# coecms/xmhw

Measured on AMD Instinct MI355X. Metric: grid-cells/sec for threshold() on 40yr daily SST, higher is better.
Workload: dtype f32 in / f64 out; 1 GPU; 0.25deg global (configs[2]): 1036800 cells per step, 1982-2021 (T=14610), windowHalfWidth=5, pctile=90, smoothPercentileWidth=31, nan_frac=0.0, skipna=False; cells_rank0=1036800, T=14610, D=366, kernel=clim_sorted_f32 (sorted row-lists in LDS, 2 lanes per cell, layout 40), slabs=1, gather=none

## Files before the change

### include/xmhw_amd.h

```cpp
#ifndef XMHW_AMD_H
#define XMHW_AMD_H

#include <stddef.h>
#include <stdint.h>

#ifdef __cplusplus
extern "C" {
#endif

#define XMHW_OK 0
#define XMHW_ERR_INVALID 1
#define XMHW_ERR_HIP 2
#define XMHW_ERR_UNSUPPORTED 3
#define XMHW_ERR_NOMEM 4
#define XMHW_ERR_COMM 5

#define XMHW_KERNEL_AUTO 0
#define XMHW_KERNEL_RING 1
#define XMHW_KERNEL_GENERIC 2

int xmhw_version(void);
const char *xmhw_arch(void);
const char *xmhw_last_error(void);
int xmhw_device_count(int *count);
// ... 72 lines not shown
    XMHW_LAYOUT_RING2_4LANE = 10,
    XMHW_LAYOUT_RING2_16LANE = 12,
    XMHW_LAYOUT_RING3_8LANE = 20,
    XMHW_LAYOUT_RING3_4LANE = 21,
    XMHW_LAYOUT_RING3_2LANE = 22,
    XMHW_LAYOUT_SORTED = 40
};
int xmhw_plan_set_layout(xmhw_plan *plan, int32_t layout);
int xmhw_plan_layout_in_use(const xmhw_plan *plan, int32_t *layout);
int xmhw_sorted_device_ok(int32_t *holds);
int xmhw_plan_set_ring2(xmhw_plan *plan, int32_t variant);
int xmhw_plan_ring2_in_use(const xmhw_plan *plan, int32_t *variant);
int xmhw_plan_f64_mode(const xmhw_plan *plan, int32_t *variant);
enum { XMHW_ROUTE_GENERIC = 0, XMHW_ROUTE_RING1 = 1, XMHW_ROUTE_RING2 = 2, XMHW_ROUTE_RING3 = 3, XMHW_ROUTE_RING4 = 4,
       XMHW_ROUTE_SORTED = 5 };
#define XMHW_ROUTE_WORDS 25
int xmhw_plan_route(const xmhw_plan *plan, int32_t elem_bytes, double q, int64_t C, int32_t *out, int32_t n);

int xmhw_clim_raw_f32(xmhw_plan *plan, const float *ts_dev, int64_t C, int64_t ld,
                      double q, int negate, double *thresh_dev, double *seas_dev,
                      int64_t ldo, void *stream);
int xmhw_clim_raw_f64(xmhw_plan *plan, const double *ts_dev, int64_t C, int64_t ld,
                      double q, int negate, double *thresh_dev, double *seas_dev,
                      int64_t ldo, void *stream);
int xmhw_clim_raw_i16(xmhw_plan *plan, const int16_t *codes_dev, int64_t C, int64_t ld, int big_endian,
                      int has_scale, double scale_factor, double add_offset, int has_fill, int32_t fill_code,
                      int decoded_itemsize, double q, int negate, double *thresh_dev, double *seas_dev,
                      int64_t ldo, void *stream);

int xmhw_clim_finish(const xmhw_plan *plan, const double *thresh_in_dev,
                     const double *seas_in_dev, int64_t C, int64_t ldo, int feb29_fix,
                     int smooth, int smooth_width, double *thresh_out_dev,
                     double *seas_out_dev, void *stream);

int xmhw_clim_f32(const float *ts_dev, const int32_t *doy_host, int64_t T, int64_t C,
                  int32_t D, int32_t window_half_width, double q, int smooth,
                  int smooth_width, int feb29_fix, int negate, double *thresh_dev,
                  double *seas_dev, void *stream);
int xmhw_clim_f64(const double *ts_dev, const int32_t *doy_host, int64_t T, int64_t C,
                  int32_t D, int32_t window_half_width, double q, int smooth,
                  int smooth_width, int feb29_fix, int negate, double *thresh_dev,
                  double *seas_dev, void *stream);
int xmhw_clim_host_f32(const float *ts_host, const int32_t *doy_host, int64_t T, int64_t C,
                       int32_t D, int32_t window_half_width, double q, int smooth,
                       int smooth_width, int feb29_fix, int negate, double *thresh_host,
                       double *seas_host);
int xmhw_clim_host_f64(const double *ts_host, const int32_t *doy_host, int64_t T, int64_t C,
                       int32_t D, int32_t window_half_width, double q, int smooth,
                       int smooth_width, int feb29_fix, int negate, double *thresh_host,
                       double *seas_host);

int xmhw_land_mask_f32(const float *ts_dev, int64_t T, int64_t C, int64_t ld, int anynans,
                       uint8_t *keep_dev, void *stream);
int xmhw_land_mask_f64(const double *ts_dev, int64_t T, int64_t C, int64_t ld, int anynans,
                       uint8_t *keep_dev, void *stream);

int xmhw_land_mask_i16(const int16_t *codes_dev, int64_t T, int64_t C, int64_t ld, int big_endian, int has_fill,
                       int32_t fill_code, int anynans, uint8_t *keep_dev, void *stream);

int xmhw_gather_cells_f32(const float *in_dev, int64_t rows, int64_t ld_in,
                          const int64_t *index_dev, int64_t n, float *out_dev, int64_t ld_out,
                          void *stream);
int xmhw_gather_cells_f64(const double *in_dev, int64_t rows, int64_t ld_in,
                          const int64_t *index_dev, int64_t n, double *out_dev, int64_t ld_out,
                          void *stream);
int xmhw_gather_cells_i16(const int16_t *in_dev, int64_t rows, int64_t ld_in,
// ... 436 lines not shown
```

### xmhw_amd/csrc/capi.cpp

```cpp
#include "../../include/xmhw_amd.h"

#include <hip/hip_runtime.h>
#include <unistd.h>

#include <cerrno>
#include <cmath>

#include <algorithm>
#include <cstdio>
#include <cstdlib>
#include <atomic>
#include <cstring>
#include <map>
#include <memory>
#include <mutex>
#include <new>
#include <string>
#include <vector>

#include "kernels.h"
#include "plan.h"
#include "route.h"
#include "stage_blocks.h"

// ... 1702 lines not shown
        pk.s = scale_factor;
        pk.o = add_offset;
        pk.val_neg = negate ? 1 : 0;
        kneg = (negate ? 1 : 0) ^ (scale_factor < 0.0 ? 1 : 0);
    }
    pk.key_neg = kneg;
    Ready rd;
    const int rc = ensure(plan, route, C, true, &rd);
    if (rc != XMHW_OK) return rc;
    hipStream_t st = static_cast<hipStream_t>(stream);
    const xmhw::Plan& h = plan->host;
    const hipError_t e = timed_launch(rd, st, [&] {
        return xmhw::launch_sorted_i16(codes, pk, C, ld, h.T, rd.table[0], rd.dev.sflags_s, rd.dev.chunks_s, rd.dev.nchunks_s, h.w,
                                       route.launch[0].tpl, h.ntracks, q, kneg, thresh, seas, ldo, st);
    });
    if (e != hipSuccess) return hip_fail(e, "packed climatology launch");
    return XMHW_OK;
}

int xmhw_clim_finish(const xmhw_plan* plan, const double* thresh_in, const double* seas_in, int64_t C,
                     int64_t ldo, int feb29_fix, int smooth, int smooth_width, double* thresh_out,
                     double* seas_out, void* stream) {
    if (!plan) return fail(XMHW_ERR_INVALID, "plan is NULL");
    if (smooth && (smooth_width <= 0 || smooth_width % 2 == 0))
        return fail(XMHW_ERR_INVALID, "Running average window should be odd");
    if (C < 0 || ldo < C) return fail(XMHW_ERR_INVALID, "bad C/ldo");
    if (C == 0) return XMHW_OK;
    if (!thresh_in || !seas_in || !thresh_out || !seas_out)
        return fail(XMHW_ERR_INVALID, "NULL device buffer");
    if (thresh_in == thresh_out || seas_in == seas_out)
        return fail(XMHW_ERR_INVALID, "in and out may not alias");
    const xmhw::Plan& h = plan->host;
    ScratchRef flags;
    if (smooth && smooth_width == 31)
        if (int rc = claim_scratch(static_cast<hipStream_t>(stream), static_cast<size_t>(C), &flags)) return rc;
    return status_of(xmhw::launch_finish(thresh_in, seas_in, C, ldo, h.D, row_index(h, 59), row_index(h, 60),
                                         row_index(h, 61), feb29_fix, smooth, smooth ? smooth_width : 1, thresh_out,
                                         seas_out, static_cast<hipStream_t>(stream), static_cast<uint8_t*>(flags.get())),
                     "clim_finish launch");
}

int xmhw_clim_f32(const float* ts, const int32_t* doy, int64_t T, int64_t C, int32_t D, int32_t w,
                  double q, int smooth, int smooth_w, int feb29_fix, int negate, double* thresh,
                  double* seas, void* stream) {
    return clim_oneshot<float>(ts, doy, T, C, D, w, q, smooth, smooth_w, feb29_fix, negate, thresh, seas,
                               stream);
}
int xmhw_clim_f64(const double* ts, const int32_t* doy, int64_t T, int64_t C, int32_t D, int32_t w,
                  double q, int smooth, int smooth_w, int feb29_fix, int negate, double* thresh,
                  double* seas, void* stream) {
    return clim_oneshot<double>(ts, doy, T, C, D, w, q, smooth, smooth_w, feb29_fix, negate, thresh, seas,
                                stream);
}
int xmhw_clim_host_f32(const float* ts, const int32_t* doy, int64_t T, int64_t C, int32_t D, int32_t w,
                       double q, int smooth, int smooth_w, int feb29_fix, int negate, double* thresh,
                       double* seas) {
    return clim_host<float>(ts, doy, T, C, D, w, q, smooth, smooth_w, feb29_fix, negate, thresh, seas);
}
int xmhw_clim_host_f64(const double* ts, const int32_t* doy, int64_t T, int64_t C, int32_t D, int32_t w,
                       double q, int smooth, int smooth_w, int feb29_fix, int negate, double* thresh,
                       double* seas) {
    return clim_host<double>(ts, doy, T, C, D, w, q, smooth, smooth_w, feb29_fix, negate, thresh, seas);
}

int xmhw_land_mask_f32(const float* ts, int64_t T, int64_t C, int64_t ld, int anynans, uint8_t* keep,
                       void* stream) {
    if (C < 0 || ld < C || T <= 0) return fail(XMHW_ERR_INVALID, "bad T/C/ld");
    return status_of(xmhw::launch_land_mask<float>(ts, T, C, ld, anynans, keep, static_cast<hipStream_t>(stream)),
                     "land_mask launch");
}
int xmhw_land_mask_f64(const double* ts, int64_t T, int64_t C, int64_t ld, int anynans, uint8_t* keep,
                       void* stream) {
// ... 847 lines not shown
```

### xmhw_amd/csrc/kernels.h

```cpp
#pragma once
#include <hip/hip_runtime.h>
#include <stdint.h>

namespace xmhw {

struct DevChunk { int32_t warm_start, begin, end; };
struct PackedI16 {
    int32_t mode = 0;
    int32_t fill = 0x7FFFFFFF;
    int32_t swap = 0;
    int32_t key_neg = 0;
    int32_t val_neg = 0;
    float sf = 1.0f, of = 0.0f;
    double s = 1.0, o = 0.0;
};
struct DevSortedChunk { int32_t warm_start, begin, end, trow0; uint32_t direct_lo, direct_hi; };

template <typename T>
hipError_t launch_generic(const T* ts, int64_t Tn, int64_t C, int64_t ld, const int32_t* row_ptr,
                          const int32_t* centres, int32_t D, int32_t w, double q, int negate,
                          double* thresh, double* seas, int64_t ldo, hipStream_t stream,
                          const uint32_t* run_flag = nullptr);

bool ring_supported(int32_t w, int32_t yps, int32_t subs, int elem_bytes);
// ... 48 lines not shown
                             int64_t ldo, hipStream_t stream);

int32_t ring4_pick_yps(int32_t w, int32_t ntracks, int32_t subs);
bool ring4_supported(int32_t w, int32_t yps, int32_t subs);
bool ring4_stats_built();
hipError_t launch_ring4_f32(const float* ts, int64_t C, int64_t ld, int64_t Tn, const uint32_t* table,
                            const uint32_t* sflags, int32_t step_min, const DevChunk* chunks, int32_t nchunks,
                            int32_t w, int32_t yps, int32_t subs, int32_t ntracks, double q, int negate,
                            double* thresh, double* seas, int64_t ldo, hipStream_t stream,
                            unsigned long long* stats = nullptr);

bool ring3_x64_supported(int32_t w, int32_t yps, int32_t subs);
hipError_t launch_ring3_f64(const double* ts, int64_t C, int64_t ld, int64_t Tn, const uint32_t* table,
                            const uint32_t* sflags, int32_t step_min, const DevChunk* chunks, int32_t nchunks,
                            int32_t w, int32_t yps, int32_t subs, int32_t ntracks, double q, int negate, double* thresh,
                            double* seas, int64_t ldo, hipStream_t stream, const uint32_t* run_flag);
bool ring3_narrowing_supported(int32_t w, int32_t yps, int32_t subs);
hipError_t launch_ring3_f32_narrowing(const double* ts, int64_t C, int64_t ld, int64_t Tn, const uint32_t* table,
                                      const uint32_t* sflags, int32_t step_min, const DevChunk* chunks,
                                      int32_t nchunks, int32_t w, int32_t yps, int32_t subs, int32_t ntracks, double q,
                                      int negate, double* thresh, double* seas, int64_t ldo, hipStream_t stream,
                                      uint32_t* narrow_flag);

hipError_t launch_ring_f32_narrowing(const double* ts, int64_t Tn, int64_t C, int64_t ld, const uint32_t* table,
                                     int32_t step_min, const DevChunk* chunks, int32_t nchunks, int32_t w,
                                     int32_t yps, int32_t subs, double q, int negate, double* thresh, double* seas,
                                     int64_t ldo, hipStream_t stream, unsigned long long* stats,
                                     uint32_t* narrow_flag);

hipError_t launch_finish(const double* th_in, const double* se_in, int64_t C, int64_t ldo, int32_t D,
                         int32_t i59, int32_t i60, int32_t i61, int feb29_fix, int smooth,
                         int32_t width, double* th_out, double* se_out, hipStream_t stream,
                         uint8_t* flags = nullptr);

template <typename T>
hipError_t launch_land_mask(const T* ts, int64_t Tn, int64_t C, int64_t ld, int anynans,
                            uint8_t* keep, hipStream_t stream);

hipError_t launch_land_mask_i16(const int16_t* codes, int64_t Tn, int64_t C, int64_t ld, int16_t fill_raw, int anynans,
                                uint8_t* keep, hipStream_t stream);

template <typename T>
hipError_t launch_gather_cells(const T* in, int64_t rows, int64_t ld_in, const int64_t* index, int64_t n,
                               T* out, int64_t ld_out, hipStream_t stream);
hipError_t launch_scatter_cells(const double* in, int64_t rows, int64_t ld_in, const int64_t* index,
                                int64_t n, double* out, int64_t ld_out, int64_t ncols_out,
                                hipStream_t stream);

template <typename T>
hipError_t launch_detect(const T* ts, int64_t Tn, int64_t C, int64_t ld, const double* thresh, int64_t ldt,
                         const int32_t* row_of_t, int32_t min_duration, int32_t join_gaps, int32_t max_gap,
                         int32_t negate, int32_t* events, int32_t* start, int32_t* end, uint8_t* bthresh,
                         int64_t ldo, int32_t* nevents, hipStream_t stream);

hipError_t launch_count_events(const int32_t* start, int64_t Tn, int64_t C, int64_t ldo, int32_t* nevents,
                               hipStream_t stream);

constexpr int kEventColumns = 31;
template <typename T>
hipError_t launch_event_stats(const T* ts, int64_t Tn, int64_t C, int64_t ld, const double* seas,
                              const double* thresh, int64_t ldc, const int32_t* row_of_t, int32_t negate,
                              const int32_t* events, int64_t ldo, const int64_t* offsets, double* table,
                              hipStream_t stream);

hipError_t launch_floor_to_f32(const double* th, int64_t rows, int64_t cols, int64_t ldi, float* out, int64_t ldo,
                               hipStream_t stream);
// ... 313 lines not shown
```

### xmhw_amd/csrc/kernels_generic.hip

```cpp
#include "device_common.h"
#include "kernels.h"
#include "packed_src.h"

namespace xmhw {

template <typename Src>
__device__ __forceinline__ void generic_cell_row(const Src& src, int64_t c, int64_t Tn, int64_t ld,
                                                 const int32_t* __restrict__ row_ptr,
                                                 const int32_t* __restrict__ centres, int32_t row, int32_t w, double q,
                                                 int negate, double& th_out, double& se_out) {
    using T = typename Src::sample;
    using K = typename KeyOf<T>::type;
    const int32_t cb = row_ptr[row], ce = row_ptr[row + 1];

    uint32_t n = 0;
    double sum = 0.0;
    for (int32_t i = cb; i < ce; ++i) {
        const int64_t t0 = centres[i];
        for (int32_t k = -w; k <= w; ++k) {
            const int64_t t = t0 + k;
            if (t < 0 || t >= Tn) continue;
            T v = src.at(c + t * ld);
            if (negate) v = -v;
            if (v == v) { ++n; sum += static_cast<double>(v); }
        }
    }
    double th = make_nan(), se = make_nan();
    if (n > 0) {
        const double vi = static_cast<double>(n - 1) * q;
        const double fl = floor(vi);
        const uint32_t lo = static_cast<uint32_t>(fl);
        const double g = vi - fl;
// ... 52 lines not shown
    generic_cell_row(PlainSrc<T>{ts}, c, Tn, ld, row_ptr, centres, row, w, q, negate, th, se);
    thresh[static_cast<int64_t>(row) * ldo + c] = th;
    seas[static_cast<int64_t>(row) * ldo + c] = se;
}

template <typename T>
hipError_t launch_generic(const T* ts, int64_t Tn, int64_t C, int64_t ld, const int32_t* row_ptr,
                          const int32_t* centres, int32_t D, int32_t w, double q, int negate,
                          double* thresh, double* seas, int64_t ldo, hipStream_t stream,
                          const uint32_t* run_flag) {
    if (C <= 0 || D <= 0) return hipSuccess;
    dim3 grid(static_cast<unsigned>((C + 255) / 256), static_cast<unsigned>(D));
    hipLaunchKernelGGL(clim_generic<T>, grid, dim3(256), 0, stream, ts, Tn, C, ld, row_ptr, centres, w,
                       q, negate, thresh, seas, ldo, run_flag);
    return hipGetLastError();
}
template hipError_t launch_generic<float>(const float*, int64_t, int64_t, int64_t, const int32_t*,
                                          const int32_t*, int32_t, int32_t, double, int, double*,
                                          double*, int64_t, hipStream_t, const uint32_t*);
template hipError_t launch_generic<double>(const double*, int64_t, int64_t, int64_t, const int32_t*,
                                           const int32_t*, int32_t, int32_t, double, int, double*,
                                           double*, int64_t, hipStream_t, const uint32_t*);

struct FinishCol {
    const double* in;
    int64_t ld;
    int32_t i60;
    double f60;
    bool sub60;
    __device__ __forceinline__ double raw(int32_t d) const { return in[static_cast<int64_t>(d) * ld]; }
    __device__ __forceinline__ double val(int32_t d) const { return (sub60 && d == i60) ? f60 : raw(d); }
};

__global__ __launch_bounds__(256) void clim_finish(const double* __restrict__ th_in,
                                                   const double* __restrict__ se_in, int64_t C,
                                                   int64_t ld, int32_t D, int32_t i59, int32_t i60,
                                                   int32_t i61, int feb29_fix, int smooth, int32_t width,
                                                   double* __restrict__ th_out,
                                                   double* __restrict__ se_out,
                                                   const uint8_t* __restrict__ only) {
    const int64_t c = static_cast<int64_t>(blockIdx.x) * blockDim.x + threadIdx.x;
    if (c >= C) return;
    if (only != nullptr && only[c] == 0) return;
    const double* in = (blockIdx.y == 0 ? th_in : se_in) + c;
    double* out = (blockIdx.y == 0 ? th_out : se_out) + c;

    int32_t nnan = 0;
    for (int32_t d = 0; d < D; ++d) {
        const double v = in[static_cast<int64_t>(d) * ld];
        nnan += (v != v) ? 1 : 0;
    }
    FinishCol col{in, ld, i60, 0.0, false};
    if (feb29_fix && i60 >= 0) {
        const double v60 = col.raw(i60);
        if (v60 == v60) {
            double s = v60;
            int32_t m = 1;
            if (i59 >= 0) { const double v = col.raw(i59); if (v == v) { s += v; ++m; } }
            if (i61 >= 0) { const double v = col.raw(i61); if (v == v) { s += v; ++m; } }
            if (m == 3) s = (col.raw(i59) + v60) + col.raw(i61);
            else if (m == 2 && i59 >= 0 && col.raw(i59) == col.raw(i59)) s = col.raw(i59) + v60;
            col.f60 = s / static_cast<double>(m);
            col.sub60 = true;
        }
    }
    const int32_t h = (width - 1) / 2;
    const double inv = static_cast<double>(width);
    if (!smooth) {
        for (int32_t d = 0; d < D; ++d) out[static_cast<int64_t>(d) * ld] = col.val(d);
        return;
    }
    if (nnan == 0) {
        int32_t trail = ((-h) % D + D) % D;
        int32_t lead = trail;
        double s = -0.0;
        for (int32_t i = 0; i < width; ++i) {
            s += col.val(lead);
            if (i + 1 < width) lead = (lead + 1 == D) ? 0 : lead + 1;
        }
// ... 40 lines not shown
    for (int32_t i = 0; i < width; ++i) {
        s += col.val(lead);
        if (i + 1 < width) lead = next_present(lead);
    }
    double fresh = -0.0;
    int32_t nfresh = 0;
    int32_t cur = first;
    for (int32_t d = 0; d < first; ++d) out[static_cast<int64_t>(d) * ld] = make_nan();
    for (int32_t j = 0; j < np; ++j) {
        out[static_cast<int64_t>(cur) * ld] = s / inv;
        s -= col.val(trail);
        trail = next_present(trail);
        lead = next_present(lead);
        const double v = col.val(lead);
        s += v;
        fresh += v;
        if (++nfresh == width) {
            s = fresh;
            fresh = -0.0;
            nfresh = 0;
        } else if (!(fabs(s) <= 1.7976931348623157e308)) {
            s = 0.0;
            for (int32_t i = 0, k = trail; i < width; ++i, k = next_present(k)) s += col.val(k);
        }
        const int32_t nxt = next_present(cur);
        if (j + 1 < np)
            for (int32_t d = cur + 1; d < nxt; ++d) out[static_cast<int64_t>(d) * ld] = make_nan();
        else
            for (int32_t d = cur + 1; d < D; ++d) out[static_cast<int64_t>(d) * ld] = make_nan();
        cur = nxt;
    }
}

template <int CT>
__global__ __launch_bounds__(256) void clim_finish_tiled(const double* __restrict__ th_in,
                                                         const double* __restrict__ se_in, int64_t C,
                                                         int64_t ld, int32_t D, int32_t i59, int32_t i60,
                                                         int32_t i61, int feb29_fix, int smooth,
                                                         int32_t width, double* __restrict__ th_out,
                                                         double* __restrict__ se_out) {
    extern __shared__ __attribute__((aligned(16))) unsigned char smem[];
    double* tile = reinterpret_cast<double*>(smem);
    int* nan_count = reinterpret_cast<int*>(smem + sizeof(double) * static_cast<size_t>(D) * CT);
    constexpr int PARTS = 256 / CT;
    const int tc = threadIdx.x % CT;
    const int part = threadIdx.x / CT;
    const int64_t cell0 = static_cast<int64_t>(blockIdx.x) * CT;
    const int64_t c = cell0 + tc;
    const bool ok = c < C;
    const double* in = (blockIdx.y == 0 ? th_in : se_in);
    double* out = (blockIdx.y == 0 ? th_out : se_out);

    if (threadIdx.x < CT) nan_count[threadIdx.x] = 0;
    __syncthreads();
    int local_nan = 0;
    for (int32_t d = part; d < D; d += PARTS) {
        const double v = ok ? in[static_cast<int64_t>(d) * ld + c] : make_nan();
        tile[d * CT + tc] = v;
        local_nan += (v != v) ? 1 : 0;
    }
    if (local_nan) atomicAdd(&nan_count[tc], local_nan);
    __syncthreads();
    if (!ok) return;
    const int nnan = nan_count[tc];

    auto raw = [&](int32_t d) { return tile[d * CT + tc]; };
// ... 73 lines not shown
    int32_t lead = trail;
    double s = -0.0;
    for (int32_t i = 0; i < width; ++i) {
        s += val(lead);
        if (i + 1 < width) lead = next_present(lead);
    }
    double fresh = -0.0;
    int32_t nfresh = 0;
    int32_t cur = first;
    for (int32_t d = 0; d < first; ++d) out[static_cast<int64_t>(d) * ld + c] = make_nan();
    for (int32_t j = 0; j < np; ++j) {
        out[static_cast<int64_t>(cur) * ld + c] = s / wd;
        s -= val(trail);
        trail = next_present(trail);
        lead = next_present(lead);
        const double v = val(lead);
        s += v;
        fresh += v;
        if (++nfresh == width) {
            s = fresh;
            fresh = -0.0;
            nfresh = 0;
        } else if (!(fabs(s) <= 1.7976931348623157e308)) {
            s = 0.0;
            for (int32_t i = 0, k = trail; i < width; ++i, k = next_present(k)) s += val(k);
        }
        const int32_t nxt = next_present(cur);
        const int32_t stop = (j + 1 < np) ? nxt : D;
        for (int32_t d = cur + 1; d < stop; ++d) out[static_cast<int64_t>(d) * ld + c] = make_nan();
        cur = nxt;
    }
}

template <int W, int A>
__global__ __launch_bounds__(256) void clim_finish_stream(const double* __restrict__ th_in,
                                                          const double* __restrict__ se_in, int64_t C, int64_t ld,
                                                          int32_t D, int32_t i59, int32_t i60, int32_t i61,
                                                          int feb29_fix, int32_t rows_per_part,
                                                          double* __restrict__ th_out, double* __restrict__ se_out,
                                                          uint8_t* __restrict__ flags) {
    constexpr int H = (W - 1) / 2;
    constexpr int U = (W % A == 0) ? W : W * A;
    static_assert(A >= 1 && (W % A == 0 || A == 2 || A == 4), "prefetch depth: 1, 2, 4 or a divisor of W");
    const int64_t c = static_cast<int64_t>(blockIdx.x) * blockDim.x + threadIdx.x;
    if (c >= C) return;
    const double* in = (blockIdx.z == 0 ? th_in : se_in) + c;
    double* out = (blockIdx.z == 0 ? th_out : se_out) + c;
    const int32_t d0 = static_cast<int32_t>(blockIdx.y) * rows_per_part;
    const int32_t d1 = d0 + rows_per_part < D ? d0 + rows_per_part : D;
    if (d0 >= d1) return;
    bool bad = false;
    const bool fix = feb29_fix && i60 >= 0;
    auto enter = [&](double v, int32_t row) -> double {
        bad = bad || (v != v);
        if (fix && row == i60 && v == v) {
            const double v59 = i59 >= 0 ? in[static_cast<int64_t>(i59) * ld] : make_nan();
            const double v61 = i61 >= 0 ? in[static_cast<int64_t>(i61) * ld] : make_nan();
            const bool p59 = v59 == v59, p61 = v61 == v61;
            double sum = p59 ? v59 + v : v;
            if (p61) sum += v61;
            v = sum / static_cast<double>(1 + (p59 ? 1 : 0) + (p61 ? 1 : 0));
        }
        return v;
    };
    auto next = [&](int32_t r) -> int32_t { return (r + 1 == D) ? 0 : r + 1; };
    double win[W], pre[A];
    int32_t r = d0 - H;
    if (r < 0) r += D;
    const int32_t r_first = r;
#pragma unroll
    for (int k = 0; k < W; ++k) {
        win[k] = in[static_cast<int64_t>(r) * ld];
        r = next(r);
    }
    int32_t r_enter = r;
#pragma unroll
    for (int k = 0; k < A; ++k) {
        pre[k] = in[static_cast<int64_t>(r) * ld];
        r = next(r);
    }
    {
        int32_t rw = r_first;
#pragma unroll
        for (int k = 0; k < W; ++k) {
            win[k] = enter(win[k], rw);
            rw = next(rw);
        }
    }
    const double wd = static_cast<double>(W);
    double s = 0.0;
    for (int32_t base = d0; base < d1; base += U) {
#pragma unroll
        for (int u = 0; u < U; ++u) {
            const int k = u % W, a = u % A;
            const int32_t d = base + u;
            if (d < d1) {
                if (k == 0) {
                    s = win[0];
#pragma unroll
                    for (int i = 1; i < W; ++i) s += win[i];
                }
                const double mean = s / wd;
                const double nv = enter(pre[a], r_enter);
                r_enter = next(r_enter);
                if (d + A < d1 - 1) pre[a] = in[static_cast<int64_t>(r) * ld];
                r = next(r);
                out[static_cast<int64_t>(d) * ld] = mean;
                s -= win[k];
                win[k] = nv;
                s += nv;
                if (!(fabs(s) <= 1.7976931348623157e308)) {
                    s = 0.0;
#pragma unroll
                    for (int i = 1; i <= W; ++i) s += win[(k + i) % W];
                }
            }
        }
    }
    if (bad) flags[c] = 1;
}

hipError_t launch_finish(const double* th_in, const double* se_in, int64_t C, int64_t ldo, int32_t D,
                         int32_t i59, int32_t i60, int32_t i61, int feb29_fix, int smooth,
                         int32_t width, double* th_out, double* se_out, hipStream_t stream, uint8_t* flags) {
    if (C <= 0 || D <= 0) return hipSuccess;
    if (smooth && width == 31 && D >= 64 && flags != nullptr) {
        hipError_t e = hipMemsetAsync(flags, 0, static_cast<size_t>(C), stream);
        if (e != hipSuccess) return e;
        const int32_t nparts = D > 732 ? 4 : 1;
        const int32_t rpp = ((D + nparts - 1) / nparts + 30) / 31 * 31;
        dim3 grid(static_cast<unsigned>((C + 255) / 256), static_cast<unsigned>((D + rpp - 1) / rpp), 2);
        hipLaunchKernelGGL((clim_finish_stream<31, 31>), grid, dim3(256), 0, stream, th_in, se_in, C, ldo, D, i59, i60, i61,
                           feb29_fix, rpp, th_out, se_out, flags);
        dim3 grid2(static_cast<unsigned>((C + 255) / 256), 2);
        hipLaunchKernelGGL(clim_finish, grid2, dim3(256), 0, stream, th_in, se_in, C, ldo, D, i59, i60, i61,
                           feb29_fix, smooth, width, th_out, se_out, static_cast<const uint8_t*>(flags));
        return hipGetLastError();
    }
    const size_t budget = 64 * 1024;
    if (static_cast<size_t>(D) * 16 * 8 + 64 <= budget) {
        dim3 grid(static_cast<unsigned>((C + 15) / 16), 2);
        hipLaunchKernelGGL(clim_finish_tiled<16>, grid, dim3(256), static_cast<size_t>(D) * 16 * 8 + 64, stream,
                           th_in, se_in, C, ldo, D, i59, i60, i61, feb29_fix, smooth, width, th_out, se_out);
    } else {
        dim3 grid(static_cast<unsigned>((C + 255) / 256), 2);
        hipLaunchKernelGGL(clim_finish, grid, dim3(256), 0, stream, th_in, se_in, C, ldo, D, i59, i60, i61,
                           feb29_fix, smooth, width, th_out, se_out, static_cast<const uint8_t*>(nullptr));
    }
    return hipGetLastError();
}

template <typename T, bool FILL>
__global__ __launch_bounds__(256) void land_mask(const T* __restrict__ ts, int64_t Tn, int64_t C,
                                                 int64_t ld, int anynans, uint8_t* __restrict__ keep, T fillv) {
    constexpr int kAhead = 8;
    __shared__ unsigned int part_nan[4][64];
    const int lane = threadIdx.x & 63, part = threadIdx.x >> 6;
    const int64_t c = static_cast<int64_t>(blockIdx.x) * 64 + lane;
    const int64_t cc = c < C ? c : C - 1;
    const int64_t t0 = Tn * part / 4, t1 = Tn * (part + 1) / 4;
    unsigned int nnan = 0;
    const T* col = ts + cc;
    int64_t t = t0;
    for (; t + kAhead <= t1; t += kAhead) {
        T v[kAhead];
#pragma unroll
        for (int u = 0; u < kAhead; ++u) v[u] = col[(t + u) * ld];
#pragma unroll
        for (int u = 0; u < kAhead; ++u) nnan += (FILL ? v[u] == fillv : v[u] != v[u]) ? 1u : 0u;
    }
    for (; t < t1; ++t) {
        const T v = col[t * ld];
        nnan += (FILL ? v == fillv : v != v) ? 1u : 0u;
    }
    part_nan[part][lane] = nnan;
    __syncthreads();
    if (part == 0 && c < C) {
        const int64_t total = static_cast<int64_t>(part_nan[0][lane]) + part_nan[1][lane] + part_nan[2][lane] + part_nan[3][lane];
// ... 169 lines not shown
```

### xmhw_amd/csrc/pybind.cpp

```cpp
#include "pybind_common.h"

PYBIND11_MODULE(_xmhw_hip, m) {
    m.doc() = "C-ABI bindings of the gfx950 xmhw threshold() path";
    auto& hip_error = py::register_exception<HipError>(m, "HipError");
    py::register_exception<Unsupported>(m, "Unsupported", hip_error.ptr());
    py::register_exception<InvalidError>(m, "InvalidArgument");
    py::register_exception<CommError>(m, "CommError");

    m.attr("KERNEL_AUTO") = XMHW_KERNEL_AUTO;
    m.attr("KERNEL_RING") = XMHW_KERNEL_RING;
    m.attr("KERNEL_GENERIC") = XMHW_KERNEL_GENERIC;

    m.def("version", &xmhw_version);
    m.def("arch", []() { return std::string(xmhw_arch()); });
    m.def("device_count", []() { int n = 0; check(xmhw_device_count(&n)); return n; });
    m.def("set_device", [](int d) { check(xmhw_set_device(d)); });
    m.def("get_device", []() { int d = 0; check(xmhw_get_device(&d)); return d; });
    m.def("device_info", [](int d) {
        char name[256] = {0};
        int cus = 0;
        uint64_t bytes = 0;
        check(xmhw_device_info(d, name, sizeof(name), &cus, &bytes));
        py::dict r;
        r["name"] = std::string(name);
// ... 95 lines not shown
    m.def("plan_chunks_in_use", [](Ptr p, int64_t C) { int32_t v = 0; check(xmhw_plan_chunks_in_use(p, C, &v)); return v; });
    m.def("debug_stats_available", []() { return xmhw_debug_stats_available() != 0; });
    m.def("plan_set_layout", [](Ptr p, int layout) { check(xmhw_plan_set_layout(p, layout)); });
    m.def("plan_layout_in_use", [](Ptr p) { int32_t v = -1; check(xmhw_plan_layout_in_use(p, &v)); return v; });
    m.def("sorted_device_ok", []() { int32_t v = 0; check(xmhw_sorted_device_ok(&v)); return v != 0; });
    m.def("plan_f64_mode", [](Ptr p) { int32_t v = -1; check(xmhw_plan_f64_mode(p, &v)); return v; });
    m.def("plan_route", [](Ptr p, int elem_bytes, double q, int64_t C) {
        py::array_t<int32_t> out(XMHW_ROUTE_WORDS);
        check(xmhw_plan_route(p, elem_bytes, q, C, out.mutable_data(), XMHW_ROUTE_WORDS));
        return out;
    });

    m.def("clim_raw", [](Ptr plan, Ptr ts, int itemsize, int64_t C, int64_t ld, double q, int negate, Ptr th, Ptr se,
                         int64_t ldo, Ptr stream) {
        check(by_itemsize(itemsize, xmhw_clim_raw_f32, xmhw_clim_raw_f64, plan, ts, C, ld, q, negate, th, se, ldo, stream));
    }, py::arg("plan"), py::arg("ts"), py::arg("itemsize"), py::arg("C"), py::arg("ld"), py::arg("q"),
       py::arg("negate"), py::arg("thresh"), py::arg("seas"), py::arg("ldo"), py::arg("stream") = 0);

    m.def("clim_raw_i16", [](Ptr plan, Ptr codes, int64_t C, int64_t ld, int big_endian, int has_scale, double scale_factor,
                             double add_offset, int has_fill, int32_t fill_code, int decoded_itemsize, double q, int negate,
                             Ptr th, Ptr se, int64_t ldo, Ptr stream) {
        check(xmhw_clim_raw_i16(plan, codes, C, ld, big_endian, has_scale, scale_factor, add_offset, has_fill, fill_code,
                                decoded_itemsize, q, negate, th, se, ldo, stream));
    }, py::arg("plan"), py::arg("codes"), py::arg("C"), py::arg("ld"), py::arg("big_endian"), py::arg("has_scale"),
       py::arg("scale_factor"), py::arg("add_offset"), py::arg("has_fill"), py::arg("fill_code"), py::arg("decoded_itemsize"),
       py::arg("q"), py::arg("negate"), py::arg("thresh"), py::arg("seas"), py::arg("ldo"), py::arg("stream") = 0);

    m.def("clim_finish", [](Ptr plan, Ptr th_in, Ptr se_in, int64_t C, int64_t ldo, int feb29_fix, int smooth, int width,
                            Ptr th_out, Ptr se_out, Ptr stream) {
        check(xmhw_clim_finish(plan, th_in, se_in, C, ldo, feb29_fix, smooth, width, th_out, se_out, stream));
    }, py::arg("plan"), py::arg("thresh_in"), py::arg("seas_in"), py::arg("C"), py::arg("ldo"),
       py::arg("feb29_fix"), py::arg("smooth"), py::arg("width"), py::arg("thresh_out"), py::arg("seas_out"),
       py::arg("stream") = 0);

    m.def("clim_host", [](py::array ts, i32arr doy, int D, int w, double q, int smooth, int smooth_w, int feb29_fix,
                          int negate) {
        if (ts.ndim() != 2) throw InvalidError("ts must be (T, C)");
        if (!(ts.flags() & py::array::c_style)) throw InvalidError("ts must be C-contiguous");
        if (ts.shape(0) != doy.size()) throw InvalidError("doy length must equal T");
        const int64_t T = ts.shape(0), C = ts.shape(1);
        py::array_t<double> th({static_cast<py::ssize_t>(D), static_cast<py::ssize_t>(C)});
        py::array_t<double> se({static_cast<py::ssize_t>(D), static_cast<py::ssize_t>(C)});
        int rc;
        if (ts.dtype().is(py::dtype::of<float>())) {
            py::gil_scoped_release r;
            rc = xmhw_clim_host_f32(static_cast<const float*>(ts.data()), doy.data(), T, C, D, w, q, smooth, smooth_w,
                                    feb29_fix, negate, th.mutable_data(), se.mutable_data());
        } else if (ts.dtype().is(py::dtype::of<double>())) {
            py::gil_scoped_release r;
            rc = xmhw_clim_host_f64(static_cast<const double*>(ts.data()), doy.data(), T, C, D, w, q, smooth, smooth_w,
                                    feb29_fix, negate, th.mutable_data(), se.mutable_data());
        } else {
            throw InvalidError("ts dtype must be float32 or float64");
        }
        check(rc);
        return py::make_tuple(th, se);
    });

    m.def("land_mask", [](Ptr ts, int itemsize, int64_t T, int64_t C, int64_t ld, int anynans, Ptr keep, Ptr stream) {
        check(by_itemsize(itemsize, xmhw_land_mask_f32, xmhw_land_mask_f64, ts, T, C, ld, anynans, keep, stream));
    }, py::arg("ts"), py::arg("itemsize"), py::arg("T"), py::arg("C"), py::arg("ld"), py::arg("anynans"),
       py::arg("keep"), py::arg("stream") = 0);
    m.def("land_mask_i16", [](Ptr codes, int64_t T, int64_t C, int64_t ld, int big_endian, int has_fill, int32_t fill_code,
                              int anynans, Ptr keep, Ptr stream) {
        check(xmhw_land_mask_i16(codes, T, C, ld, big_endian, has_fill, fill_code, anynans, keep, stream));
    }, py::arg("codes"), py::arg("T"), py::arg("C"), py::arg("ld"), py::arg("big_endian"), py::arg("has_fill"),
// ... 408 lines not shown
```

### xmhw_amd/device.py

```python
import os as _os
import sys
import threading as _threading
import time as _time
from concurrent.futures import ThreadPoolExecutor
from contextlib import contextmanager

import numpy as np

from ._lib import hip
from .exception import XmhwException

KERNELS = {"auto": 0, "ring": 1, "generic": 2}


class PackedArray(np.ndarray):

    def __new__(cls, array, decode):
        obj = np.asarray(array).view(cls)
        obj.decode = dict(decode)
        return obj

    def __array_finalize__(self, obj):
        if obj is not None:
            self.decode = getattr(obj, "decode", None)
# ... 237 lines not shown
            self.handle = 0

    def __del__(self):
        try:
            self.destroy()
        except Exception:
            pass


def _first_family(route):
    return route["launches"][0]["family"] if route["launches"] else None


def clim_raw(plan, ts_dev, itemsize, C, q, negate, thresh_dev, seas_dev, ld=None, ldo=None, stream=0):
    with as_xmhw_errors():
        hip().clim_raw(plan.handle, _ptr(ts_dev), itemsize, C, C if ld is None else ld, float(q), int(bool(negate)),
                       _ptr(thresh_dev), _ptr(seas_dev), C if ldo is None else ldo, stream)


def clim_raw_packed(plan, codes_dev, C, q, negate, thresh_dev, seas_dev, scale_factor=None, add_offset=None, fill=None,
                    decoded="float32", big_endian=False, ld=None, ldo=None, stream=0):
    has_scale = scale_factor is not None or add_offset is not None
    with as_xmhw_errors(also="HipError"):
        hip().clim_raw_i16(plan.handle, _ptr(codes_dev), C, C if ld is None else ld, int(bool(big_endian)), int(has_scale),
                           1.0 if scale_factor is None else float(scale_factor), 0.0 if add_offset is None else float(add_offset),
                           int(fill is not None), 0 if fill is None else int(fill), 8 if str(decoded) in ("float64", "f64", "8") else 4,
                           float(q), int(bool(negate)), _ptr(thresh_dev), _ptr(seas_dev), C if ldo is None else ldo, stream)


def clim_finish(plan, th_in, se_in, C, feb29_fix, smooth, width, th_out, se_out, ldo=None, stream=0):
    with as_xmhw_errors():
        hip().clim_finish(plan.handle, _ptr(th_in), _ptr(se_in), C, C if ldo is None else ldo, int(bool(feb29_fix)),
                          int(bool(smooth)), int(width), _ptr(th_out), _ptr(se_out), stream)


def _clim_on_device(scope, plan, d_ts, isz, n, q, negate, finish, raw=None, out=None, recipe=None):
    raw_th, raw_se = raw or (scope.alloc(8 * plan.D * n), scope.alloc(8 * plan.D * n))
    if recipe is not None:
        clim_raw_packed(plan, d_ts, n, q, negate, raw_th, raw_se, scale_factor=recipe["scale"], add_offset=recipe["offset"],
                        fill=recipe["fill"], decoded=recipe["decoded"], big_endian=recipe["big_endian"])
    else:
        clim_raw(plan, d_ts, isz, n, q, negate, raw_th, raw_se)
    if finish is None:
        return raw_th, raw_se
    out_th, out_se = out or (scope.alloc(8 * plan.D * n), scope.alloc(8 * plan.D * n))
    clim_finish(plan, raw_th, raw_se, n, *finish, out_th, out_se)
    return out_th, out_se


def calc_clim_device(ts, doy, pctile, windowHalfWidth, smoothPercentile, smoothPercentileWidth,
                     tstep, coldSpells=False, kernel="auto", nchunks=0, max_batch_bytes=32 << 30,
                     narrowing=True, pad=None):
    ts = native_float(ts)
    if ts.ndim != 2:
        raise XmhwException("calc_clim_device expects a (time, cell) array")
    T, C = ts.shape
    h = hip()
    plan = Plan(doy, windowHalfWidth, kernel=kernel, nchunks=nchunks, narrowing=narrowing)
    try:
        with DeviceScope() as s:
            D = plan.D
            th = np.empty((D, C), dtype=np.float64)
            se = np.empty((D, C), dtype=np.float64)
            if C == 0:
                return plan.doys.copy(), th, se
            isz = ts.dtype.itemsize
# ... 477 lines not shown
```

Before: 43.84 million cells/s.

## Fuse smoothing finish into single stream launch with LDS wraparound and inline fallback

Adds a single-launch variant of the streaming 31-day smoothing kernel for the clim_finish step. The first 30 wraparound rows are kept in LDS instead of being re-read from global memory, and bad (NaN) columns are handled inline by the generic per-column finish rather than through a flags buffer, memset and second launch. This removes the scratch claim, the memset and the extra pass, at the cost of 60 KB of LDS per block, which may lower occupancy. It also adds an env toggle and a last-path query for diagnostics.

```diff
diff --git a/include/xmhw_amd.h b/include/xmhw_amd.h
--- a/include/xmhw_amd.h
+++ b/include/xmhw_amd.h
@@ -128,6 +128,7 @@
                      const double *seas_in_dev, int64_t C, int64_t ldo, int feb29_fix,
                      int smooth, int smooth_width, double *thresh_out_dev,
                      double *seas_out_dev, void *stream);
+int xmhw_clim_finish_last_path(int32_t *path);
 
 int xmhw_clim_f32(const float *ts_dev, const int32_t *doy_host, int64_t T, int64_t C,
                   int32_t D, int32_t window_half_width, double q, int smooth,
diff --git a/xmhw_amd/csrc/capi.cpp b/xmhw_amd/csrc/capi.cpp
--- a/xmhw_amd/csrc/capi.cpp
+++ b/xmhw_amd/csrc/capi.cpp
@@ -1758,12 +1758,18 @@
         return fail(XMHW_ERR_INVALID, "in and out may not alias");
     const xmhw::Plan& h = plan->host;
     ScratchRef flags;
-    if (smooth && smooth_width == 31)
+    if (smooth && smooth_width == 31 && !xmhw::finish_one_launch(h.D, smooth, smooth_width))
         if (int rc = claim_scratch(static_cast<hipStream_t>(stream), static_cast<size_t>(C), &flags)) return rc;
     return status_of(xmhw::launch_finish(thresh_in, seas_in, C, ldo, h.D, row_index(h, 59), row_index(h, 60),
                                          row_index(h, 61), feb29_fix, smooth, smooth ? smooth_width : 1, thresh_out,
                                          seas_out, static_cast<hipStream_t>(stream), static_cast<uint8_t*>(flags.get())),
                      "clim_finish launch");
+}
+
+int xmhw_clim_finish_last_path(int32_t* path) {
+    if (!path) return fail(XMHW_ERR_INVALID, "NULL argument");
+    *path = xmhw::finish_last_path();
+    return XMHW_OK;
 }
 
 int xmhw_clim_f32(const float* ts, const int32_t* doy, int64_t T, int64_t C, int32_t D, int32_t w,
diff --git a/xmhw_amd/csrc/kernels.h b/xmhw_amd/csrc/kernels.h
--- a/xmhw_amd/csrc/kernels.h
+++ b/xmhw_amd/csrc/kernels.h
@@ -104,6 +104,9 @@
                          int32_t i59, int32_t i60, int32_t i61, int feb29_fix, int smooth,
                          int32_t width, double* th_out, double* se_out, hipStream_t stream,
                          uint8_t* flags = nullptr);
+bool finish_one_launch(int32_t D, int smooth, int32_t width);
+enum FinishPath : int32_t { kFinishNone = 0, kFinishStream = 1, kFinishOne = 2, kFinishTiled = 3, kFinishUntiled = 4 };
+int32_t finish_last_path();
 
 template <typename T>
 hipError_t launch_land_mask(const T* ts, int64_t Tn, int64_t C, int64_t ld, int anynans,
diff --git a/xmhw_amd/csrc/kernels_generic.hip b/xmhw_amd/csrc/kernels_generic.hip
--- a/xmhw_amd/csrc/kernels_generic.hip
+++ b/xmhw_amd/csrc/kernels_generic.hip
@@ -1,3 +1,6 @@
+#include <atomic>
+#include <cstdlib>
+
 #include "device_common.h"
 #include "kernels.h"
 #include "packed_src.h"
@@ -116,19 +119,9 @@
     __device__ __forceinline__ double val(int32_t d) const { return (sub60 && d == i60) ? f60 : raw(d); }
 };
 
-__global__ __launch_bounds__(256) void clim_finish(const double* __restrict__ th_in,
-                                                   const double* __restrict__ se_in, int64_t C,
-                                                   int64_t ld, int32_t D, int32_t i59, int32_t i60,
-                                                   int32_t i61, int feb29_fix, int smooth, int32_t width,
-                                                   double* __restrict__ th_out,
-                                                   double* __restrict__ se_out,
-                                                   const uint8_t* __restrict__ only) {
-    const int64_t c = static_cast<int64_t>(blockIdx.x) * blockDim.x + threadIdx.x;
-    if (c >= C) return;
-    if (only != nullptr && only[c] == 0) return;
-    const double* in = (blockIdx.y == 0 ? th_in : se_in) + c;
-    double* out = (blockIdx.y == 0 ? th_out : se_out) + c;
-
+__device__ __forceinline__ void finish_column(const double* __restrict__ in, double* __restrict__ out, int64_t ld,
+                                              int32_t D, int32_t i59, int32_t i60, int32_t i61, int feb29_fix,
+                                              int smooth, int32_t width) {
     int32_t nnan = 0;
     for (int32_t d = 0; d < D; ++d) {
         const double v = in[static_cast<int64_t>(d) * ld];
@@ -235,6 +228,20 @@
     }
 }
 
+__global__ __launch_bounds__(256) void clim_finish(const double* __restrict__ th_in,
+                                                   const double* __restrict__ se_in, int64_t C,
+                                                   int64_t ld, int32_t D, int32_t i59, int32_t i60,
+                                                   int32_t i61, int feb29_fix, int smooth, int32_t width,
+                                                   double* __restrict__ th_out,
+                                                   double* __restrict__ se_out,
+                                                   const uint8_t* __restrict__ only) {
+    const int64_t c = static_cast<int64_t>(blockIdx.x) * blockDim.x + threadIdx.x;
+    if (c >= C) return;
+    if (only != nullptr && only[c] == 0) return;
+    finish_column((blockIdx.y == 0 ? th_in : se_in) + c, (blockIdx.y == 0 ? th_out : se_out) + c, ld, D, i59, i60, i61,
+                  feb29_fix, smooth, width);
+}
+
 template <int CT>
 __global__ __launch_bounds__(256) void clim_finish_tiled(const double* __restrict__ th_in,
                                                          const double* __restrict__ se_in, int64_t C,
@@ -374,7 +381,7 @@
     }
 }
 
-template <int W, int A>
+template <int W, int A, bool ONE = false>
 __global__ __launch_bounds__(256) void clim_finish_stream(const double* __restrict__ th_in,
                                                           const double* __restrict__ se_in, int64_t C, int64_t ld,
                                                           int32_t D, int32_t i59, int32_t i60, int32_t i61,
@@ -384,6 +391,12 @@
     constexpr int H = (W - 1) / 2;
     constexpr int U = (W % A == 0) ? W : W * A;
     static_assert(A >= 1 && (W % A == 0 || A == 2 || A == 4), "prefetch depth: 1, 2, 4 or a divisor of W");
+    static_assert(!ONE || (W % 2 == 1 && A >= 1), "one part: an odd window");
+    double (*keep)[256] = nullptr;
+    if constexpr (ONE) {
+        __shared__ double wrap_rows[W - 1][256];
+        keep = wrap_rows;
+    }
     const int64_t c = static_cast<int64_t>(blockIdx.x) * blockDim.x + threadIdx.x;
     if (c >= C) return;
     const double* in = (blockIdx.z == 0 ? th_in : se_in) + c;
@@ -425,10 +438,12 @@
         int32_t rw = r_first;
 #pragma unroll
         for (int k = 0; k < W; ++k) {
+            if (ONE && k < W - 1) keep[k][threadIdx.x] = win[k];
             win[k] = enter(win[k], rw);
             rw = next(rw);
         }
     }
+    [[maybe_unused]] const int32_t keep_from = d1 - 1 - A - (W - 1);
     const double wd = static_cast<double>(W);
     double s = 0.0;
     for (int32_t base = d0; base < d1; base += U) {
@@ -445,7 +460,10 @@
                 const double mean = s / wd;
                 const double nv = enter(pre[a], r_enter);
                 r_enter = next(r_enter);
-                if (d + A < d1 - 1) pre[a] = in[static_cast<int64_t>(r) * ld];
+                if (d + A < d1 - 1) {
+                    if (ONE && d >= keep_from) pre[a] = keep[d - keep_from][threadIdx.x];
+                    else pre[a] = in[static_cast<int64_t>(r) * ld];
+                }
                 r = next(r);
                 out[static_cast<int64_t>(d) * ld] = mean;
                 s -= win[k];
@@ -459,14 +477,41 @@
             }
         }
     }
-    if (bad) flags[c] = 1;
-}
+    if (ONE) {
+        if (bad) finish_column(in, out, ld, D, i59, i60, i61, feb29_fix, 1, W);
+    } else {
+        if (bad) flags[c] = 1;
+    }
+}
+
+static bool finish_wide_enabled() {
+    static const bool on = [] {
+        const char* v = std::getenv("XMHW_FINISH_WIDE");
+        return !(v && v[0] == '0' && v[1] == '\0');
+    }();
+    return on;
+}
+
+bool finish_one_launch(int32_t D, int smooth, int32_t width) {
+    return smooth && width == 31 && D >= 64 && finish_wide_enabled();
+}
+
+static std::atomic<int32_t> last_finish_path{kFinishNone};
+int32_t finish_last_path() { return last_finish_path.load(std::memory_order_relaxed); }
 
 hipError_t launch_finish(const double* th_in, const double* se_in, int64_t C, int64_t ldo, int32_t D,
                          int32_t i59, int32_t i60, int32_t i61, int feb29_fix, int smooth,
                          int32_t width, double* th_out, double* se_out, hipStream_t stream, uint8_t* flags) {
     if (C <= 0 || D <= 0) return hipSuccess;
+    if (finish_one_launch(D, smooth, width)) {
+        dim3 grid(static_cast<unsigned>((C + 255) / 256), 1, 2);
+        hipLaunchKernelGGL((clim_finish_stream<31, 31, true>), grid, dim3(256), 0, stream, th_in, se_in, C, ldo, D, i59, i60,
+                           i61, feb29_fix, D, th_out, se_out, static_cast<uint8_t*>(nullptr));
+        last_finish_path.store(kFinishOne, std::memory_order_relaxed);
+        return hipGetLastError();
+    }
     if (smooth && width == 31 && D >= 64 && flags != nullptr) {
+        last_finish_path.store(kFinishStream, std::memory_order_relaxed);
         hipError_t e = hipMemsetAsync(flags, 0, static_cast<size_t>(C), stream);
         if (e != hipSuccess) return e;
         const int32_t nparts = D > 732 ? 4 : 1;
@@ -482,10 +527,12 @@
     const size_t budget = 64 * 1024;
     if (static_cast<size_t>(D) * 16 * 8 + 64 <= budget) {
         dim3 grid(static_cast<unsigned>((C + 15) / 16), 2);
+        last_finish_path.store(kFinishTiled, std::memory_order_relaxed);
         hipLaunchKernelGGL(clim_finish_tiled<16>, grid, dim3(256), static_cast<size_t>(D) * 16 * 8 + 64, stream,
                            th_in, se_in, C, ldo, D, i59, i60, i61, feb29_fix, smooth, width, th_out, se_out);
     } else {
         dim3 grid(static_cast<unsigned>((C + 255) / 256), 2);
+        last_finish_path.store(kFinishUntiled, std::memory_order_relaxed);
         hipLaunchKernelGGL(clim_finish, grid, dim3(256), 0, stream, th_in, se_in, C, ldo, D, i59, i60, i61,
                            feb29_fix, smooth, width, th_out, se_out, static_cast<const uint8_t*>(nullptr));
     }
diff --git a/xmhw_amd/csrc/pybind.cpp b/xmhw_amd/csrc/pybind.cpp
--- a/xmhw_amd/csrc/pybind.cpp
+++ b/xmhw_amd/csrc/pybind.cpp
@@ -151,6 +151,8 @@
     }, py::arg("plan"), py::arg("thresh_in"), py::arg("seas_in"), py::arg("C"), py::arg("ldo"),
        py::arg("feb29_fix"), py::arg("smooth"), py::arg("width"), py::arg("thresh_out"), py::arg("seas_out"),
        py::arg("stream") = 0);
+
+    m.def("_clim_finish_last_path", []() { int32_t v = 0; check(xmhw_clim_finish_last_path(&v)); return v; });
 
     m.def("clim_host", [](py::array ts, i32arr doy, int D, int w, double q, int smooth, int smooth_w, int feb29_fix,
                           int negate) {
diff --git a/xmhw_amd/device.py b/xmhw_amd/device.py
--- a/xmhw_amd/device.py
+++ b/xmhw_amd/device.py
@@ -293,6 +293,10 @@
     with as_xmhw_errors():
         hip().clim_finish(plan.handle, _ptr(th_in), _ptr(se_in), C, C if ldo is None else ldo, int(bool(feb29_fix)),
                           int(bool(smooth)), int(width), _ptr(th_out), _ptr(se_out), stream)
+
+
+def clim_finish_last_path():
+    return int(hip()._clim_finish_last_path())
 
 
 def _clim_on_device(scope, plan, d_ts, isz, n, q, negate, finish, raw=None, out=None, recipe=None):
```

After: 44.18 million cells/s (median of 4 runs). Within noise of the previous version (+0.8%).
